# wns349/tensorflow-yolo

Hardware: AMD Instinct MI355X
Metric: images/sec at 1/2/4/8 MI355X + post-NMS box-set match vs CPU ref (higher is better)
Workload: dtype f16; 1 GPU; v3-608-b32-fp16; network=v3, batch_per_gpu=32, global_batch=32, weights=seeded synthetic Darknet stream (random-init), streams=1

## Files before the change

### tensorflow-yolo_amd/csrc/api.cpp

```cpp
#include <cstdio>
#include <cstring>
#include <new>

#include <cmath>
#include "yolo_internal.h"

namespace yolo {
const char *get_error();
}
using namespace yolo;

#define HIP_TRY(expr)                                                                          \
    do {                                                                                       \
        hipError_t e_ = (expr);                                                                \
        if (e_ != hipSuccess) {                                                                \
            set_error(std::string(#expr) + ": " + hipGetErrorString(e_));                      \
            return YOLO_ERR_HIP;                                                               \
        }                                                                                      \
    } while (0)

static int fail(int code, const std::string &msg) {
    set_error(msg);
    return code;
}
// ... 181 lines not shown
    }
    int esz(const View &v) const { return v.f32 ? 4 : net->esize; }
    unsigned char *view_ptr(const View &v) const { return buf_base(v.buf) + (size_t)(v.base + v.coff) * esz(v); }
};

void conv_vec_flags(const yolo_net *net, const Kernel &k, bool out_f32, int &vec_out, int &vec_res) {
    const int epc = net->epc;
    const int ch = k.cfg == CFG_N32 ? 8 : 16;
    const int oepc = out_f32 ? 4 : epc;
    vec_out = (k.cout % ch == 0) && (k.out.ld % oepc == 0) && ((k.out.base + k.out.coff) % oepc == 0) && (k.out.img_stride % oepc == 0);
    vec_res = k.has_res && (k.cout % ch == 0) && (k.in2.ld % epc == 0) && (k.in2.coff % epc == 0) && (k.in2.img_stride % epc == 0);
}

int make_conv_params(yolo_net *net, const Kernel &k, const Ptrs &P, int batch, ConvParams &p) {
    const int dtype = net->opt.dtype;
    memset(&p, 0, sizeof p);
    const View &in = k.in;
    const long long in_bytes = (long long)batch * in.img_stride * net->esize;
    if (in_bytes > 0x7ffffff0LL)
        return fail(YOLO_ERR_ARG, "conv input tensor exceeds 2 GiB (32-bit buffer addressing): lower the batch");
    p.in = P.buf_base(in.buf);
    p.in_bytes = (uint32_t)in_bytes;
    p.wgt = weights_at(net, k.w_off);
    p.wgt_bytes = (uint32_t)k.w_bytes;
    p.bias = reinterpret_cast<const float *>(weights_at(net, k.b_off));
    p.H = in.H; p.W = in.W; p.in_ld = in.ld; p.in_coff = in.coff; p.in_img_stride = in.img_stride;
    const yolo_layer_desc &d = net->layers[k.src_layer].d;
    const int Ho = net->layers[k.src_layer].H, Wo = net->layers[k.src_layer].W;
    p.Ho = Ho; p.Wo = Wo; p.HoWo = Ho * Wo;
    const long long M = (long long)batch * Ho * Wo;
    if (M > 0x7fffffffLL) return fail(YOLO_ERR_ARG, "too many output pixels for one launch");
    p.M = (int)M;
    p.Cout = k.cout;
    p.out = P.view_ptr(k.out);
    p.out_ld = k.out.ld;
    p.out_img_stride = k.out.img_stride;
    p.out_f32 = k.out.f32 || dtype == YOLO_DTYPE_F32;
    {
        const long long ob = (long long)batch * k.out.img_stride * (p.out_f32 ? 4 : net->esize);
        p.out_bytes = ob > 0 && ob <= 0x7ffffff0LL ? (uint32_t)ob : 0u;
    }
    p.ksize = d.ksize; p.stride = d.stride; p.pad = (d.ksize - 1) / 2; p.taps = d.ksize * d.ksize;
    p.ktiles = k.ktiles;
    p.tiles_per_tap = k.perchunk ? 1 : k.cpt / 8;
    p.cin_chunks = k.cpt;
    p.cpt_shift = k.cpt == 1 ? 0 : k.cpt == 2 ? 1 : 2;
    p.wrow_bytes = (uint32_t)k.ktiles * 128;
    p.leaky = k.leaky; p.outmode = k.outmode; p.has_res = k.has_res;
    p.f32 = dtype == YOLO_DTYPE_F32;
    int vo = 0, vr = 0;
    conv_vec_flags(net, k, p.out_f32 != 0, vo, vr);
    p.vec_out = vo && ((uintptr_t)P.buf_base(k.out.buf) % 16 == 0);
    if (k.head && net->obj_bytes && net->head.n_classes > 0 && !p.vec_out && p.out_f32 && k.outmode == OUT_NORMAL && !k.has_res) {
        const int width = 5 + net->head.n_classes;
        const long long base = k.out.base + k.out.coff;
        const size_t rows = net->out_count / (size_t)width;
        if (k.out.ld % width == 0 && base % width == 0 && rows * width == net->out_count && (size_t)batch * rows * 4 <= net->obj_bytes) {
            p.obj_out = reinterpret_cast<float *>(net->dev_ws + net->obj_off) + (size_t)P.img0 * rows;
            p.obj_width = width; p.obj_rows = (int)rows; p.obj_row0 = (int)(base / width); p.obj_na = k.out.ld / width;
            p.obj_min = net->obj_min_logit;
        }
    }
    if (k.has_res) {
        p.res = P.view_ptr(k.in2);
        p.res_ld = k.in2.ld;
        p.res_img_stride = k.in2.img_stride;
        const long long rbytes = (long long)batch * k.in2.img_stride * net->esize;
        p.res_bytes = rbytes > 0 && rbytes <= 0x7ffffff0LL ? (uint32_t)rbytes : 0u;
        p.vec_res = vr;
    }
    return YOLO_OK;
}

bool dma_eligible(const yolo_net *net, const Kernel &k) {
    if (k.cpt % 4) return false;
    return net->opt.dtype == YOLO_DTYPE_F16 || (k.ksize == 3 && k.stride == 1);
}
bool conv_tile_valid(const yolo_net *net, const Kernel &k, int tile) {
    if (k.outmode == OUT_POOL2 && tile != 12 && tile != 13 && tile != 17) return false;
    if (tile == 0) return true;
    if (net->opt.dtype == YOLO_DTYPE_F32 && !dma_cfg_f32_ok(tile)) return false;
    if ((tile == 18 || tile == 21 || tile == 22) && k.in.H != k.in.W) return false;
    if ((tile == 20 || tile == 21 || tile == 23) && ((k.in.H & 1) || net->opt.dtype != YOLO_DTYPE_F16)) return false;
    return dma_eligible(net, k) && dma_cfg_valid(tile, k.cout, k.cpt, true, k.ksize, k.stride, k.in.W);
}

int choose_ksplit(const Kernel &k, const ConvParams &p, int tile, size_t slab_bytes, int &ku) {
    ku = 0;
    if (!slab_bytes || p.M <= 0) return 1;
    long long blocks;
    int units, min_units;
    if (tile == 0) {
        const int na = k.cfg == CFG_N128 ? 128 : k.cfg == CFG_N64 ? 64 : 32, nb = k.cfg == CFG_N128 ? 128 : 256;
        blocks = ((long long)p.M + nb - 1) / nb * ((p.Cout + na - 1) / na);
        units = p.ktiles;
        min_units = 2;
    } else if (dma_cfg_is_tap(tile) && dma_cfg_splitk_ok(tile)) {
        const long long mq = (long long)(p.M / p.HoWo) * (p.H + 1) * (p.W + 1);
        blocks = (mq + dma_cfg_nb(tile) - 1) / dma_cfg_nb(tile) * ((p.Cout + dma_cfg_na(tile) - 1) / dma_cfg_na(tile));
        units = p.cin_chunks >> 2;
        min_units = 2;
    } else {
        return 1;
    }
    if (blocks > 128 || units < 2 * min_units) return 1;
    const long long kmax = units / min_units < 32 ? units / min_units : 32;
    long long ks = 512 / blocks;
    if (ks > kmax) ks = 256 / blocks;
    if (ks > kmax) ks = kmax;
    const size_t cout_pad = ((size_t)p.Cout + 127) / 128 * 128;
    const size_t wbytes = (size_t)p.Cout * (size_t)p.taps * (size_t)p.cin_chunks * 16;
    const size_t small_cap = (size_t)(p.taps == 1 ? 24 : (p.f32 || units >= 8) ? 16 : 8) << 20;
    while (ks >= 2 && ((size_t)ks * (size_t)p.M * cout_pad * 4 > slab_bytes || (size_t)ks * (size_t)p.M * cout_pad * 4 > (2 * wbytes > small_cap ? 2 * wbytes : small_cap))) --ks;
    if (ks < 2) return 1;
    ku = (int)((units + ks - 1) / ks);
    return (units + ku - 1) / ku;
}

struct ConvPick { int tile, ks, ku, pair; };
const size_t kSplitkSlabMax = (size_t)64 << 20;

ConvPick pick_conv(const yolo_net *net, const Kernel &k, const ConvParams &p, int tile_req, size_t slab_bytes) {
    int tile = tile_req;
    if (!dma_eligible(net, k) || (tile > 0 && !conv_tile_valid(net, k, tile))) tile = 0;
    else if (tile < 0) {
        tile = choose_dma_cfg(p.M, k.cout, k.cpt, p.taps, k.has_res, true, k.stride, k.in.W, net->opt.dtype == YOLO_DTYPE_F32);
        if (tile == 18 && !conv_tile_valid(net, k, 18)) tile = conv_tile_valid(net, k, 15) ? 15 : 8;
        if (tile == 22 && !conv_tile_valid(net, k, 22)) tile = conv_tile_valid(net, k, 10) ? 10 : 8;
        if ((tile == 20 || tile == 21) && !conv_tile_valid(net, k, tile)) tile = conv_tile_valid(net, k, 20) ? 20 : conv_tile_valid(net, k, 5) ? 5 : 0;
        if (tile == 23 && !conv_tile_valid(net, k, 23)) tile = conv_tile_valid(net, k, 6) ? 6 : 0;
    }
    static const bool no_pair_w = getenv("YOLO_NO_PAIR_SPLIT") != nullptr;
    bool wide_pair = false;
    if (tile > 0 && dma_cfg_is_tap(tile) && !no_pair_w && tile_req <= 0 && !p.f32 && (p.cin_chunks >> 2) >= 8 && p.HoWo > 0) {
        const long long mq = (long long)(p.M / p.HoWo) * (p.H + 1) * (p.W + 1);
        const long long ct = (p.Cout + 127) / 128;
        const long long b8 = (mq + 255) / 256 * ct, b22 = (long long)(p.M / p.HoWo) * ct;
        wide_pair = (conv_tile_valid(net, k, 22) && b22 >= 64 && b22 <= 128 && (size_t)b22 * 2 * 98304 <= slab_bytes) ||
                    (conv_tile_valid(net, k, 8) && b8 >= 64 && b8 <= 128 && (size_t)b8 * 2 * 131072 <= slab_bytes);
    }
    int ku = 0;
    int ks = wide_pair ? 1 : choose_ksplit(k, p, tile, slab_bytes, ku);
    if (ks <= 1 && !wide_pair && tile_req <= 0 && tile > 0 && dma_cfg_is_tap(tile) && tile != 11 && conv_tile_valid(net, k, 11)) {
        int ku11 = 0;
        const int ks11 = choose_ksplit(k, p, 11, slab_bytes, ku11);
        if (ks11 > 1) { tile = 11; ks = ks11; ku = ku11; }
    }
    int pair = 0;
    static const bool no_pair = getenv("YOLO_NO_PAIR_SPLIT") != nullptr;
    if (ks <= 1 && tile > 0 && dma_cfg_is_tap(tile) && !no_pair && tile_req <= 0) {
        const long long mq = (long long)(p.M / p.HoWo) * (p.H + 1) * (p.W + 1);
        const int units = p.cin_chunks >> 2;
        const long long ct = (p.Cout + 127) / 128;
        const long long b8 = (mq + 255) / 256 * ct, b11 = (mq + 127) / 128 * ct;
        const long long b22 = (long long)(p.M / p.HoWo) * ct;
        if (units >= 8 && !p.f32 && conv_tile_valid(net, k, 22) && b22 >= 64 && b22 <= 128 && (size_t)b22 * 2 * 98304 <= slab_bytes) {
            tile = 22; ks = 2; ku = (units + 1) / 2; pair = 1;
        } else if (units >= 8 && !p.f32 && conv_tile_valid(net, k, 8) && b8 >= 64 && b8 <= 128 && (size_t)b8 * 2 * 131072 <= slab_bytes) {
            tile = 8; ks = 2; ku = (units + 1) / 2; pair = 1;
        } else if (units >= 8 && conv_tile_valid(net, k, 11) && b11 > 128 && b11 <= 256 && (size_t)b11 * 2 * 65536 <= slab_bytes) {
            tile = 11; ks = 2; ku = (units + 1) / 2; pair = 1;
        }
    }
    static const bool no_inl = getenv("YOLO_NO_INLAUNCH_SPLITK") != nullptr;
    if (ks > 1 && ks <= 8 && !pair && tile == 11 && !no_inl) {
        const long long mq = (long long)(p.M / p.HoWo) * (p.H + 1) * (p.W + 1);
        const long long nb11 = (mq + 127) / 128 * ((p.Cout + 127) / 128);
        if (nb11 * 128 <= (long long)kPairCounterBytes && (size_t)nb11 * (size_t)ks * 65536 <= slab_bytes) pair = 1;
    }
    return ConvPick{tile, ks, ku, pair};
}

void conv_shape_params(const yolo_net *net, const Kernel &k, int batch, ConvParams &p) {
    memset(&p, 0, sizeof p);
    const yolo_layer_desc &d = net->layers[k.src_layer].d;
    p.H = k.in.H; p.W = k.in.W;
    p.Ho = net->layers[k.src_layer].H; p.Wo = net->layers[k.src_layer].W; p.HoWo = p.Ho * p.Wo;
    p.M = (int)((long long)batch * p.HoWo);
    p.Cout = k.cout;
    p.ksize = d.ksize; p.stride = d.stride; p.taps = d.ksize * d.ksize;
    p.ktiles = k.ktiles; p.cin_chunks = k.cpt;
    p.f32 = net->opt.dtype == YOLO_DTYPE_F32;
    p.out_f32 = k.out.f32 || p.f32;
    p.outmode = k.outmode; p.has_res = k.has_res;
    conv_vec_flags(net, k, p.out_f32 != 0, p.vec_out, p.vec_res);
    const long long ob = (long long)batch * k.out.img_stride * (p.out_f32 ? 4 : net->esize);
    p.out_bytes = ob > 0 && ob <= 0x7ffffff0LL ? (uint32_t)ob : 0u;
    const long long rb = k.has_res ? (long long)batch * k.in2.img_stride * net->esize : 0;
    p.res_bytes = rb > 0 && rb <= 0x7ffffff0LL ? (uint32_t)rb : 0u;
}

size_t splitk_slab_bytes(const yolo_net *net) {
    const int per = net->arena_full ? net->opt.max_batch : (net->opt.max_batch + net->arenas - 1) / net->arenas;
    size_t need = 0;
    for (const Kernel &k : net->kernels) {
        if (k.kind != K_CONV || k.stem >= 2) continue;
        for (int b = 1; b <= per; ++b) {
            ConvParams p;
            conv_shape_params(net, k, b, p);
            const ConvPick pk = pick_conv(net, k, p, k.tile, kSplitkSlabMax);
            if (pk.pair) {
                const long long mq = (long long)(p.M / p.HoWo) * (p.H + 1) * (p.W + 1);
                const int nb = dma_cfg_nb(pk.tile);
                const long long ptiles = pk.tile == 22 ? (long long)(p.M / p.HoWo) : (mq + nb - 1) / nb;
                const size_t bytes = (size_t)(ptiles * ((p.Cout + 127) / 128)) * (size_t)pk.ks * 128 * (size_t)nb * 4;
                if (bytes > need) need = bytes;
            } else if (pk.ks > 1) {
                const size_t bytes = (size_t)pk.ks * (size_t)p.M * (size_t)((p.Cout + 127) / 128 * 128) * 4;
                if (bytes > need) need = bytes;
            }
        }
    }
    return need ? kPairCounterBytes + (need + 4095) / 4096 * 4096 : 0;
// ... 742 lines not shown
```

### tensorflow-yolo_amd/csrc/conv_dma.hip

```cpp
#include "conv_common.h"
#include <cstdio>
#include <vector>

namespace yolo {

template <int N>
__device__ __forceinline__ void wait_vmcnt() {
    asm volatile("s_waitcnt vmcnt(%0)" ::"n"(N) : "memory");
}

typedef __attribute__((address_space(3))) void lds_void;

__device__ __forceinline__ void dma16(__amdgpu_buffer_rsrc_t rsrc, unsigned char *lds_dst, uint32_t voff) {
#if defined(__HIP_DEVICE_COMPILE__)
    __builtin_amdgcn_raw_ptr_buffer_load_lds(rsrc, (lds_void *)lds_dst, 16, voff, 0, 0, 0);
#else
    (void)rsrc; (void)lds_dst; (void)voff;
#endif
}

template <int BKC>
__device__ __forceinline__ int lds_swz(int r) {
    if (BKC == 8) return (r >> 1) & 7;
    return (0x78 >> (2 * ((r >> 2) & 3))) & 3;
// ... 136 lines not shown
            else wait_vmcnt<0>();
        } else {
            if (S >= 4 && after >= 2) wait_vmcnt<2 * JB>();
            else if (S >= 3 && after >= 1) wait_vmcnt<JB>();
            else wait_vmcnt<0>();
        }
        __builtin_amdgcn_sched_barrier(0);
        __builtin_amdgcn_s_barrier();
#ifdef YOLO_EXPERIMENT
        if (p.trace && kt == 0) t_first = wall_clock64();
        if (kt + S - 1 < KT && !(p.dbg & 1)) issue_tile(kt + S - 1, fill);
        if (!(p.dbg & 2)) compute(stage);
#else
        if (kt + S - 1 < KT) issue_tile(kt + S - 1, fill);
        compute(stage);
#endif
        stage = stage + 1 == S ? 0 : stage + 1;
        fill = fill + 1 == S ? 0 : fill + 1;
    }

#ifdef YOLO_EXPERIMENT
    if (p.dbg & 4) return;
    const unsigned long long t_loop = p.trace ? wall_clock64() : 0ull;
#endif
    if constexpr (FUSE2) {
        static_assert(!FUSE2 || (WM == 2 && WN == 4 && TM == 4 && TP == 4 && 2 * LDS_BYTES <= 163840), "back-to-back 1x1: 128 x 256 tile, two per CU");
        conv_epilogue_fused_1x1<0, false>(p, acc, m0, wm, wn, wave, lane, smem);
    } else
    if constexpr (EPI == 2) {
        static_assert(8 * 16 * kStagePitch(TM) * 4 + NB * kStageFlagAnchors * 4 <= S * TILE_BYTES, "staging slabs + row flags must fit in the ring");
        __syncthreads();
        conv_epilogue_f32_staged<TM, TP, 0, true, NB>(p, acc, n0 + wm * (TM * 16), m0 + wn * (TP * 16), lane,
                                         reinterpret_cast<float *>(smem) + wave * 16 * kStagePitch(TM),
                                         reinterpret_cast<float *>(smem) + 8 * 16 * kStagePitch(TM), wn * (TP * 16));
    } else if constexpr (EPI == 1) {
        conv_epilogue_fast<TM, TP, 0>(p, acc, n0 + wm * (TM * 16) + fq * CH, m0 + wn * (TP * 16), fr);
    } else {
        conv_epilogue<T, TM, TP, 0, true>(p, acc, n0 + wm * (TM * 16) + fq * CH, m0 + wn * (TP * 16), fr);
    }
#ifdef YOLO_EXPERIMENT
    if (p.trace && tid == 0) {
        asm volatile("s_waitcnt vmcnt(0)" ::: "memory");
        unsigned long long *r = p.trace + (size_t)blockIdx.x * 8;
        r[0] = t_start; r[1] = t_setup; r[2] = t_loop; r[3] = wall_clock64();
        r[4] = __builtin_amdgcn_s_getreg(0xF804);
        r[5] = __builtin_amdgcn_s_getreg(0xF814);
        r[6] = t_first;
        r[7] = (unsigned long long)clock64() - c_start;
    }
#endif
}

struct DmaCfg {
    int na, nb, slots_per_cu;
    float rate;
    const char *name;
    int bkc;
};
static const DmaCfg kCfgs[] = {
    {128, 128, 2, 0.55f, "", 8},
    {256, 256, 1, 0.80f, "256x256,K64,S2", 8},
    {256, 128, 1, 0.85f, "256x128,K64,S3", 8},
    {128, 256, 1, 0.85f, "128x256,K64,S3", 8},
    {256, 256, 1, 1.00f, "256x256,K32,S4", 4},
    {256, 128, 2, 1.30f, "256x128,K32,S3,x2", 4},
    {128, 256, 2, 1.30f, "128x256,K32,S3,x2", 4},
    {64, 512, 2, 1.00f, "64x512,K32,S2,x2", 4},
    {128, 256, 2, 1.00f, "128x256,tap9,x2", 4},
    {256, 256, 1, 1.00f, "256x256,tap9", 4},
    {128, 192, 2, 1.00f, "128x192,tap9,x2", 4},
    {128, 128, 2, 1.00f, "128x128,tap9,x2", 4},
    {128, 256, 2, 1.00f, "128x256,tap9,2d,x2", 4},
    {64, 256, 2, 1.00f, "64x256,tap9,2d,x2", 4},
    {128, 128, 3, 1.00f, "128x128,K32,S3,x3", 4},
    {256, 224, 1, 1.00f, "256x224,tap9", 4},
    {128, 128, 3, 1.00f, "128x128,tap9,2d,x3", 4},
    {32, 256, 2, 1.00f, "32x256,tap9,2d,x2", 4},
    {128, 384, 1, 1.00f, "128x384,tap9,img", 4},
    {128, 192, 1, 1.00f, "128x192,K64,S4", 8},
    {128, 256, 2, 1.00f, "128x256,tap9,s2,x2", 4},
    {128, 384, 1, 1.00f, "128x384,tap9,s2,img", 4},
    {128, 192, 2, 1.00f, "128x192,tap9,img,x2", 4},
    {128, 256, 2, 1.00f, "128x256,tap9,s2,wide,x2", 4},
};
static const int kNumCfgs = 24;
static const int kFirstTapCfg = 8, kLastTapCfg = 13;
static inline bool is_tap_cfg(int cfg) { return (cfg >= kFirstTapCfg && cfg <= kLastTapCfg) || (cfg >= 15 && cfg <= 18) || (cfg >= 20 && cfg <= 23); }
static inline int tap_variant(int cfg) { return cfg >= 20 ? cfg - 10 : cfg >= 15 ? cfg - 9 : cfg - kFirstTapCfg; }
bool dma_cfg_is_tap(int cfg) { return is_tap_cfg(cfg); }
bool dma_cfg_f32_ok(int cfg) { return is_tap_cfg(cfg) && conv_tap_f32_ok(tap_variant(cfg)); }

bool dma_cfg_valid(int cfg, int cout, int cin_chunks, bool v1_ok, int ksize, int stride, int W) {
    if (cfg == 0) return v1_ok;
    if (cfg < 0 || cfg >= kNumCfgs) return false;
    const DmaCfg &k = kCfgs[cfg];
    if (cin_chunks % k.bkc) return false;
    if (is_tap_cfg(cfg) && (ksize != 3 || stride != (conv_tap_stride2(tap_variant(cfg)) ? 2 : 1) || !conv_tap_fits(tap_variant(cfg), W))) return false;
    if (k.na == 32) return cout <= 32 && cout > 16;
    if (k.na == 64) return cout <= 64 && (!is_tap_cfg(cfg) || cout > 32);
    return k.na <= (cout + 127) / 128 * 128 && cout > 64;
}

struct TileCost { float a_shared, a_mid, a_alone, f; };
static const TileCost kCost[] = {
    {1.14f, 1.14f, 0.82f, 9.0f},
    {1.45f, 1.45f, 1.45f, 20.0f},
    {0.82f, 0.82f, 0.82f, 12.0f},
    {0.82f, 0.82f, 0.82f, 12.0f},
    {1.47f, 1.47f, 1.47f, 20.0f},
    {1.75f, 1.75f, 1.30f, 8.0f},
    {1.75f, 1.75f, 1.30f, 8.0f},
    {0.0f, 0.0f, 0.0f, 0.0f},
    {1.20f, 1.45f, 0.76f, 7.9f},
    {1.20f, 1.20f, 1.20f, 20.0f},
    {0.94f, 1.32f, 0.68f, 8.5f},
    {0.76f, 0.90f, 0.63f, 6.9f},
    {0.90f, 1.10f, 0.60f, 17.0f},
    {1.00f, 1.00f, 0.60f, 5.8f},
    {1.10f, 1.50f, 0.70f, 8.0f},
    {1.05f, 1.05f, 1.05f, 18.0f},
    {0.0f, 0.0f, 0.0f, 0.0f},
    {0.0f, 0.0f, 0.0f, 0.0f},
    {0.90f, 0.90f, 0.90f, 18.0f},
    {0.60f, 0.60f, 0.60f, 12.0f},
    {1.20f, 1.45f, 0.76f, 7.9f},
    {0.90f, 0.90f, 0.90f, 18.0f},
    {0.94f, 1.32f, 0.68f, 8.5f},
    {0.0f, 0.0f, 0.0f, 0.0f},
};

int choose_dma_cfg(int M, int cout, int cin_chunks, int taps, int has_res, bool v1_ok, int stride, int W, bool tap_only) {
    const int ksize = taps == 9 ? 3 : 1;
#ifdef YOLO_EXPERIMENT
    const char *force = getenv("YOLO_CONV_TILE");
    if (force && *force && dma_cfg_valid(atoi(force), cout, cin_chunks, v1_ok, ksize, stride, W) && (!tap_only || atoi(force) == 0 || is_tap_cfg(atoi(force))))
        return atoi(force);
#endif
    const int fallback = v1_ok ? 0 : -1;
    if (cout <= 32 && M >= 8192 && dma_cfg_valid(17, cout, cin_chunks, v1_ok, ksize, stride, W)) return 17;
    if (cout <= 64) {
        if (M >= 8192 && dma_cfg_valid(13, cout, cin_chunks, v1_ok, ksize, stride, W)) return 13;
        return !tap_only && dma_cfg_valid(7, cout, cin_chunks, v1_ok, ksize, stride, W) && M >= 8192 ? 7 : fallback;
    }
    if (!tap_only && taps == 9 && stride == 1 && W > 110 && cout <= 128 && cin_chunks <= 8 && M >= 262144 &&
        dma_cfg_valid(12, cout, cin_chunks, v1_ok, ksize, stride, W))
        return 12;
    if (!tap_only && taps == 9 && stride == 1 && W > 110 && cout <= 128 && cin_chunks <= 8 && M >= 65536 && M < 262144 &&
        dma_cfg_valid(16, cout, cin_chunks, v1_ok, ksize, stride, W))
        return 16;
    if (tap_only && v1_ok && taps == 9 && stride == 1 && W <= 14 && taps * cin_chunks * 4 >= 4608 &&
        ((long long)M * (W + 1) * (W + 1) / ((long long)W * W) + 127) / 128 * ((cout + 127) / 128) > 512)
        return 0;
    const double k64 = taps * cin_chunks / 8.0;
    int best = fallback;
    double best_t = 1e300;
    for (int c = 0; c < kNumCfgs; ++c) {
        if (tap_only && !dma_cfg_f32_ok(c)) continue;
        if (c == 12 && W <= 110) continue;
        const long long wg128 = (long long)((M + 127) / 128) * ((cout + 127) / 128);
        if (c == 14 && taps != 1 && !(stride == 2 && wg128 > 128 && wg128 <= 256)) continue;
        if (c == 19 && taps != 1) continue;
        if (c == 7 || c == 13 || c == 16 || c == 17 || c == 23 || !dma_cfg_valid(c, cout, cin_chunks, v1_ok, ksize, stride, W)) continue;
        const DmaCfg &k = kCfgs[c];
        long long Meff = M;
        const int Wq = is_tap_cfg(c) && conv_tap_stride2(tap_variant(c)) ? W / 2 : W;
        if (is_tap_cfg(c) && conv_tap_stride2(tap_variant(c))) {
            if (cin_chunks <= 8) continue;
            Meff = (long long)M * (Wq + 1) * (Wq + 1) / ((long long)Wq * Wq);
        } else if (is_tap_cfg(c)) {
            if (conv_tap_is2d(tap_variant(c))) { const long long th = k.nb / 16, tx = (W + 15) / 16, ty = (W + th - 1) / th; Meff = (long long)M * tx * ty * k.nb / ((long long)W * W); }
            else Meff = (long long)M * (W + 1) * (W + 1) / ((long long)W * W);
        }
        long long blocks = (Meff + k.nb - 1) / k.nb * ((cout + k.na - 1) / k.na);
        if (is_tap_cfg(c) && conv_tap_image_aligned(tap_variant(c))) blocks = (long long)(M / (Wq * Wq)) * ((cout + k.na - 1) / k.na);
        if (is_tap_cfg(c) && conv_tap_stride2(tap_variant(c)) && blocks <= 128) continue;
        const long long slots = 256LL * k.slots_per_cu;
        double rounds, a;
        if (k.slots_per_cu == 1) {
            rounds = (double)((blocks + slots - 1) / slots);
            a = kCost[c].a_shared;
        } else if (blocks > slots) {
            rounds = (double)blocks / slots + 0.5;
            a = kCost[c].a_shared;
        } else {
            rounds = 1.0;
            a = blocks <= 256 ? kCost[c].a_alone : kCost[c].a_mid;
        }
        const double t = rounds * (k64 * a + kCost[c].f * (has_res ? 1.0 : 0.7));
        if (t < best_t) { best_t = t; best = c; }
    }
    return best;
}

int dma_num_cfgs() { return kNumCfgs; }
int dma_cfg_na(int cfg) { return cfg > 0 && cfg < kNumCfgs ? kCfgs[cfg].na : 128; }
int dma_cfg_nb(int cfg) { return cfg > 0 && cfg < kNumCfgs ? kCfgs[cfg].nb : 128; }
bool dma_cfg_splitk_ok(int cfg) { return is_tap_cfg(cfg) && conv_tap_splitk_ok(tap_variant(cfg)); }
int dma_cfg_bkc(int cfg) { return cfg > 0 && cfg < kNumCfgs ? kCfgs[cfg].bkc : 8; }
const char *dma_cfg_name(int cfg) { return cfg > 0 && cfg < kNumCfgs ? kCfgs[cfg].name : ""; }

#define YOLO_DMA_VARIANTS(X) \
    X(1, 2, 4, 8, 4, 2, 8, 2) \
    X(2, 4, 2, 4, 4, 3, 8, 2) \
    X(3, 2, 4, 4, 4, 3, 8, 2) \
    X(4, 2, 4, 8, 4, 4, 4, 2) \
    X(5, 4, 2, 4, 4, 3, 4, 4) \
    X(6, 2, 4, 4, 4, 3, 4, 4) \
    X(7, 1, 8, 4, 4, 2, 4, 4) \
    X(14, 2, 4, 4, 2, 3, 4, 6) \
    X(19, 2, 4, 4, 3, 4, 8, 2)

static inline int dma_epilogue_kind(const ConvParams &p) {
    if (p.out_f32 && !p.vec_out && p.outmode == OUT_NORMAL && !p.has_res) return 2;
    static const bool no_fast_epi = getenv("YOLO_NO_FAST_EPI") != nullptr;
    return !no_fast_epi && conv_fast_epilogue_ok(p) ? 1 : 0;
}

static hipError_t launch_dma_tile(const ConvParams &p, int cfg, hipStream_t s) {
    const dim3 grid((unsigned)p.n_blocks), block(512);
    if (p.fuse2) {
        if (cfg != 6 || !conv_fast_epilogue_ok(p) || p.has_res || p.n_tiles_n != 1 || p.Cout != 128 || !p.w2 || !p.b2 || !p.out2 || !p.out2_bytes) return hipErrorInvalidValue;
        hipLaunchKernelGGL((conv_igemm_dma_kernel<2, 4, 4, 4, 3, 4, 4, true>), grid, block, 0, s, p);
        return hipGetLastError();
    }
    switch (cfg) {
#define X(id, ...) case id: \
        if (dma_epilogue_kind(p) == 2) hipLaunchKernelGGL((conv_igemm_dma_kernel<__VA_ARGS__, false, 2>), grid, block, 0, s, p); \
        else if (dma_epilogue_kind(p) == 1) hipLaunchKernelGGL((conv_igemm_dma_kernel<__VA_ARGS__, false, 1>), grid, block, 0, s, p); \
        else hipLaunchKernelGGL((conv_igemm_dma_kernel<__VA_ARGS__, false, 0>), grid, block, 0, s, p); \
        break;
        YOLO_DMA_VARIANTS(X)
#undef X
    default: return hipErrorInvalidValue;
    }
    return hipGetLastError();
}

#ifdef YOLO_EXPERIMENT
static hipError_t launch_traced(ConvParams p, int cfg, hipStream_t s) {
    const char *tf = getenv("YOLO_CONV_TRACE");
    unsigned long long *dev = nullptr;
    const size_t bytes = (size_t)p.n_blocks * 64;
    if (hipMalloc((void **)&dev, bytes) != hipSuccess) return hipErrorOutOfMemory;
    (void)hipMemset(dev, 0, bytes);
    p.trace = dev;
    hipError_t e = is_tap_cfg(cfg) ? launch_conv_tap(p, tap_variant(cfg), s) : launch_dma_tile(p, cfg, s);
    if (e == hipSuccess) e = hipStreamSynchronize(s);
    std::vector<unsigned long long> host((size_t)p.n_blocks * 8);
    if (e == hipSuccess) e = hipMemcpy(host.data(), dev, bytes, hipMemcpyDeviceToHost);
    (void)hipFree(dev);
    if (e == hipSuccess) {
        if (FILE *fp = fopen(tf, "ab")) {
            const unsigned long long hdr[8] = {(unsigned long long)p.n_blocks, (unsigned long long)p.M, (unsigned long long)p.Cout,
                                               (unsigned long long)p.cin_chunks, (unsigned long long)p.H, (unsigned long long)p.W,
                                               (unsigned long long)cfg, (unsigned long long)(p.ksize * 10 + p.stride)};
            fwrite(hdr, 8, 8, fp);
            fwrite(host.data(), 8, host.size(), fp);
            fclose(fp);
        }
    }
    return e;
}
#endif

hipError_t launch_conv_dma(const ConvParams &p0, int cfg, hipStream_t s) {
    if (cfg <= 0 || cfg >= kNumCfgs) return hipErrorInvalidValue;
    ConvParams p = p0;
    const DmaCfg &k = kCfgs[cfg];
#ifdef YOLO_EXPERIMENT
    { const char *d = getenv("YOLO_CONV_DBG"); p.dbg = d ? atoi(d) : 0; }
#endif
    p.n_tiles_n = (p.Cout + k.na - 1) / k.na;
    const long long blocks = ((long long)p.M + k.nb - 1) / k.nb * p.n_tiles_n;
    if (blocks <= 0 || blocks > 0x7fffffffLL) return hipErrorInvalidValue;
    p.n_blocks = (int)blocks;
    conv_set_divisors(p, p.cin_chunks / k.bkc);
    if (is_tap_cfg(cfg)) {
        long long mq;
        if (conv_tap_is2d(tap_variant(cfg))) {
            const int th = k.nb / 16;
            p.t2_shift = th == 16 ? 8 : 7;
            if (th != 16 && th != 8) return hipErrorInvalidValue;
            p.qW = (p.W + 15) / 16;
            p.qHW = p.qW * ((p.H + th - 1) / th);
            mq = (long long)(p.M / p.HoWo) * p.qHW * k.nb;
        } else {
            p.qW = p.Wo + 1;
            p.qHW = (p.Ho + 1) * (p.Wo + 1);
            mq = (long long)(p.M / p.HoWo) * p.qHW;
        }
        const bool img = conv_tap_image_aligned(tap_variant(cfg));
        p.q_stride = img ? p.qHW : k.nb;
        const long long qblocks = img ? (long long)(p.M / p.HoWo) * p.n_tiles_n : (mq + k.nb - 1) / k.nb * p.n_tiles_n;
        if (qblocks <= 0 || qblocks > 0x7fffffffLL) return hipErrorInvalidValue;
        p.Mq = (int)mq;
        p.n_blocks = (int)qblocks;
        conv_set_divisors(p, p.cin_chunks / k.bkc);
#ifdef YOLO_EXPERIMENT
        if (getenv("YOLO_CONV_TRACE")) return launch_traced(p, cfg, s);
#endif
        p.stream = 1;
#ifdef YOLO_EXPERIMENT
        if (getenv("YOLO_NO_TAP_STREAM")) p.stream = 0;
#endif
        return launch_conv_tap(p, tap_variant(cfg), s);
    }
#ifdef YOLO_EXPERIMENT
    if (getenv("YOLO_CONV_TRACE")) return launch_traced(p, cfg, s);
#endif
    return launch_dma_tile(p, cfg, s);
}

std::string dma_cfg_symbol_for(int cfg, bool f32, const ConvParams &p) {
    if (p.fuse2) return cfg == 6 ? "void yolo::conv_igemm_dma_kernel<2, 4, 4, 4, 3, 4, 4, true, 0>(yolo::ConvParams)"
                       : cfg == 23 ? "void yolo::conv3x3_tap_kernel<false, 2, 4, 4, 4, 26, 4, 4, false, true, true>(yolo::ConvParams)"
                                   : "void yolo::conv3x3_tap_kernel<false, 2, 4, 4, 4, 27, 4, 2, false, true, true>(yolo::ConvParams)";
    if (is_tap_cfg(cfg) && conv_tap_stream_ok(p, tap_variant(cfg))) return conv_tap_stream_symbol(tap_variant(cfg));
    if (!is_tap_cfg(cfg)) {
        std::string sym = dma_cfg_symbol(cfg, f32, false);
        const size_t at = sym.rfind(", false, 0>(");
        if (at != std::string::npos) sym[at + 9] = (char)('0' + dma_epilogue_kind(p));
        return sym;
    }
    std::string sym = dma_cfg_symbol(cfg, f32, !f32 && conv_fast_epilogue_ok(p) && cfg != 20 && cfg != 23);
    if (is_tap_cfg(cfg) && p.outmode == OUT_POOL2) {
        const size_t at = sym.rfind(", 2, false, false, false>(");
        if (at != std::string::npos) sym.replace(at, 26, ", 3, false, false, false>(");
    }
    return sym;
}

const char *dma_cfg_symbol(int cfg, bool f32, bool fast) {
    if (is_tap_cfg(cfg)) return conv_tap_symbol(tap_variant(cfg), f32, fast);
    switch (cfg) {
#define X(id, ...) case id: return fast ? "void yolo::conv_igemm_dma_kernel<" #__VA_ARGS__ ", false, 1>(yolo::ConvParams)" \
                                          : "void yolo::conv_igemm_dma_kernel<" #__VA_ARGS__ ", false, 0>(yolo::ConvParams)";
        YOLO_DMA_VARIANTS(X)
#undef X
    default: return "";
    }
}

}
```

### tensorflow-yolo_amd/csrc/yolo_internal.h

```cpp
#pragma once
#include <hip/hip_runtime.h>
#include <stdint.h>
#include <string>
#include <vector>

#include "yolo_hip.h"

namespace yolo {

enum OutMode { OUT_NORMAL = 0, OUT_UP2 = 1, OUT_REORG2 = 2, OUT_POOL2 = 3 };
enum BufId { BUF_NONE = -1, BUF_USER_OUT = -2, BUF_USER_IN = -3 };
enum ConvCfg { CFG_N128 = 0, CFG_N64 = 1, CFG_N32 = 2 };
enum KernelKind { K_PREP = 0, K_CONV = 1, K_POOL = 2, K_ELTWISE = 3, K_FIRST = 4 };

struct View {
    int buf = BUF_NONE;
    int H = 0, W = 0, C = 0;
    int ld = 0;
    int coff = 0;
    long long img_stride = 0;
    long long base = 0;
    bool f32 = false;
};

// ... 138 lines not shown
    uint32_t w2_bytes, wrow2;
    int H, W, Ho, Wo, out_ld;
    long long in_img_stride, out_img_stride;
    int tiles_x, tiles_y, n_tiles;
    FastDiv dtx, dty;
};

struct ResizeParams {
    const unsigned char *src;
    float *dst;
    int src_h, src_w, src_row_bytes, dst_h, dst_w, swap_rb;
};

struct PoolParams {
    const void *in;
    void *out;
    int H, W, C, in_ld, Ho, Wo, out_ld, stride;
    long long in_img_stride, out_img_stride;
    long long total;
};

struct EltParams {
    const void *a;
    const void *b;
    void *out;
    int H, W, C, a_ld, b_ld, out_ld, outmode, out_f32, a_f32;
    long long a_img_stride, b_img_stride, out_img_stride;
    long long total;
};

struct ReduceParams {
    const float *part;
    const float *bias;
    const void *res;
    void *out;
    float *obj_out;
    int obj_width, obj_rows, obj_row0, obj_na;
    int ksplit, M, Cout, cout_pad, HoWo, Wo;
    int out_ld, res_ld, leaky, outmode, out_f32, f32;
    long long out_img_stride, res_img_stride;
};

struct DecodeScale {
    int row0, h, w, na;
    double aw[YOLO_MAX_ANCHORS], ah[YOLO_MAX_ANCHORS];
};

struct DecodeParams {
    const float *logits;
    const float *obj;
    int version, n_classes, rows, n_scales;
    DecodeScale sc[YOLO_MAX_SCALES];
    float threshold;
    int cap;
    void *cand;
    int *cand_count;
    long long total_rows;
};

struct Candidate {
    float x, y;
    double w, h;
    float prob;
    int cls;
    unsigned scan;
    int pad_;
};

struct NmsParams {
    const Candidate *cand;
    const int *cand_count;
    int *reset_count;
    int cap, max_boxes, mode;
    double iou_threshold;
    yolo_box *boxes;
    int *counts;
    int *status;
    int *keep_idx;
    unsigned char *scratch;
    size_t scratch_stride;
};

hipError_t launch_conv(const ConvParams &p, int dtype, int cfg, bool perchunk, hipStream_t s);
int choose_dma_cfg(int M, int cout, int cin_chunks, int taps, int has_res, bool v1_ok, int stride, int W, bool tap_only = false);
bool dma_cfg_valid(int cfg, int cout, int cin_chunks, bool v1_ok, int ksize, int stride, int W);
bool dma_cfg_is_tap(int cfg);
int dma_cfg_bkc(int cfg);
hipError_t launch_conv_dma(const ConvParams &p, int cfg, hipStream_t s);
hipError_t launch_conv_tap(const ConvParams &p, int variant, hipStream_t s);
bool conv_tap_stream_ok(const ConvParams &p, int variant);
bool conv_tap_fits(int variant, int W);
bool conv_tap_is2d(int variant);
bool conv_tap_stride2(int variant);
bool conv_tap_image_aligned(int variant);
bool conv_tap_f32_ok(int variant);
bool dma_cfg_f32_ok(int cfg);
const char *dma_cfg_name(int cfg);
const char *dma_cfg_symbol(int cfg, bool f32, bool fast = false);
const char *conv_tap_symbol(int variant, bool f32, bool fast = false);
std::string dma_cfg_symbol_for(int cfg, bool f32, const ConvParams &p);
const char *conv_tap_stream_symbol(int variant);
std::string conv_symbol(int dtype, int cfg, bool perchunk, bool f32_emu = false);
bool conv_f32_emu_rule(int f32_products, int dtype, const ConvParams &p, int cfg, bool perchunk, int ksplit);
std::string first_symbol(int dtype, int cout, bool pool);
std::string aux_symbol(int kind, int dtype, bool vec);
int dma_num_cfgs();
int dma_cfg_na(int cfg);
int dma_cfg_nb(int cfg);
bool dma_cfg_splitk_ok(int cfg);
hipError_t launch_splitk_reduce(const ReduceParams &p, hipStream_t s);
bool conv_tap_splitk_ok(int variant);
bool conv_tap_pair_ok(int variant, bool f32);
hipError_t launch_prep(const PrepParams &p, int dtype, hipStream_t s);
hipError_t launch_resize(const ResizeParams &p, hipStream_t s);
hipError_t launch_first(const FirstParams &p, int dtype, hipStream_t s);
hipError_t launch_stem(const StemParams &p, int batch, hipStream_t s, int max_grid = 512);
hipError_t launch_pool(const PoolParams &p, int dtype, hipStream_t s);
hipError_t launch_eltwise(const EltParams &p, int dtype, hipStream_t s);
hipError_t launch_decode(const DecodeParams &p, int batch, hipStream_t s, bool zero_counts = true);
hipError_t launch_nms(const NmsParams &p, int batch, hipStream_t s);
size_t nms_lds_bytes(int cap);
size_t nms_scratch_bytes(int cap);

struct Kernel {
    int kind = 0;
    int layer = -1;
    int src_layer = -1;
    View in, in2, out;
    int ksize = 0, stride = 0, cout = 0, cin = 0, cin_s = 0, leaky = 0, outmode = 0, has_res = 0;
    int cfg = 0, perchunk = 0, cpt = 0, ktiles = 0;
    int tile = -1;
    int head = 0;
    int pool_fused = 0;
    int stem = 0;
    int fuse2_next = 0;
    int fuse2_prev = 0;
    int side = 0;
    size_t w_off = 0, b_off = 0, w_bytes = 0;
    size_t w_src = 0;
    int batch_norm = 0;
    int pool_stride = 0;
    std::string note;
};

struct LayerInfo {
    yolo_layer_desc d;
    int H = 0, W = 0, C = 0;
    std::vector<int> consumers;
    int fused_into = -1;
    View view;
    bool materialised = false;
};

}

struct yolo_net {
    yolo_net_options opt;
    std::vector<yolo::LayerInfo> layers;
    std::vector<yolo::Kernel> kernels;
    std::vector<yolo::Buffer> buffers;
    yolo_head_desc head;
    size_t weight_count = 0;
    size_t weights_bytes = 0;
    size_t act_bytes = 0;
    size_t logits_off = 0, cand_off = 0, count_off = 0, nms_off = 0;
    size_t splitk_off = 0, splitk_bytes = 0;
    size_t obj_off = 0, obj_bytes = 0;
    bool obj_valid = false;
    int cand_clean = 0;
    int side_chains = 0;
    std::vector<hipStream_t> branch;
    std::vector<hipEvent_t> e_bfork, e_bjoin;
// ... 28 lines not shown
```

Before: 6389 images/sec.

## Add persistent LDS-resident-weight streaming kernel for large 1x1 convolutions

Introduces a persistent 1x1 convolution kernel that loads the full weight slice into LDS once per workgroup and streams input pixel tiles through a multi-stage async buffer-load ring, with epilogues overlapped against in-flight loads. The tile chooser selects it for stride-1, non-residual f16 1x1 layers where Cout matches the slice width, K exceeds 256 and there are enough pixel tiles. The goal is to remove repeated weight reloads and per-tile launch/prologue cost of the generic GEMM tiles. The fixed grid of 256 workgroups and large LDS footprint limit occupancy, and applicability is narrow.

After: 6383 images/sec (median of 3 runs). Within noise of the previous version (-0.1%).

```diff
diff --git a/tensorflow-yolo_amd/csrc/api.cpp b/tensorflow-yolo_amd/csrc/api.cpp
--- a/tensorflow-yolo_amd/csrc/api.cpp
+++ b/tensorflow-yolo_amd/csrc/api.cpp
@@ -287,6 +287,7 @@
     if (net->opt.dtype == YOLO_DTYPE_F32 && !dma_cfg_f32_ok(tile)) return false;
     if ((tile == 18 || tile == 21 || tile == 22) && k.in.H != k.in.W) return false;
     if ((tile == 20 || tile == 21 || tile == 23) && ((k.in.H & 1) || net->opt.dtype != YOLO_DTYPE_F16)) return false;
+    if (tile == 24 && (k.has_res || k.out.f32 || net->opt.dtype != YOLO_DTYPE_F16)) return false;
     return dma_eligible(net, k) && dma_cfg_valid(tile, k.cout, k.cpt, true, k.ksize, k.stride, k.in.W);
 }
 
@@ -334,6 +335,8 @@
         if (tile == 22 && !conv_tile_valid(net, k, 22)) tile = conv_tile_valid(net, k, 10) ? 10 : 8;
         if ((tile == 20 || tile == 21) && !conv_tile_valid(net, k, tile)) tile = conv_tile_valid(net, k, 20) ? 20 : conv_tile_valid(net, k, 5) ? 5 : 0;
         if (tile == 23 && !conv_tile_valid(net, k, 23)) tile = conv_tile_valid(net, k, 6) ? 6 : 0;
+        if (tile == 24 && !conv_tile_valid(net, k, 24))
+            tile = choose_dma_cfg(p.M, k.cout, k.cpt, p.taps, k.has_res, true, k.stride, k.in.W, net->opt.dtype == YOLO_DTYPE_F32, true);
     }
     static const bool no_pair_w = getenv("YOLO_NO_PAIR_SPLIT") != nullptr;
     bool wide_pair = false;
diff --git a/tensorflow-yolo_amd/csrc/conv_1x1.hip b/tensorflow-yolo_amd/csrc/conv_1x1.hip
--- /dev/null
+++ b/tensorflow-yolo_amd/csrc/conv_1x1.hip
@@ -0,0 +1,235 @@
+#include "conv_common.h"
+
+namespace yolo {
+
+typedef __attribute__((address_space(3))) void c1_lds_void;
+
+template <int N>
+__device__ __forceinline__ void c1_wait_vmcnt() {
+    asm volatile("s_waitcnt vmcnt(%0)" ::"n"(N) : "memory");
+}
+
+__device__ __forceinline__ void c1_dma16(__amdgpu_buffer_rsrc_t rsrc, unsigned char *lds_dst, uint32_t voff) {
+#if defined(__HIP_DEVICE_COMPILE__)
+    __builtin_amdgcn_raw_ptr_buffer_load_lds(rsrc, (c1_lds_void *)lds_dst, 16, voff, 0, 0, 0);
+#else
+    (void)rsrc; (void)lds_dst; (void)voff;
+#endif
+}
+
+__device__ __forceinline__ int c1_swz(int r) { return (0x78 >> (2 * ((r >> 2) & 3))) & 3; }
+
+constexpr int kC1LdsBytes = 163840;
+constexpr int kC1Grid = 256;
+constexpr int kC1MaxSlices = 4;
+
+template <int WM, int WN, int TM, int TP, int S, int EPI>
+__global__ void __launch_bounds__(512, 2) conv1x1_stream_kernel(const ConvParams p) {
+    typedef _Float16 T;
+    static_assert(WM * WN == 8, "eight waves per workgroup");
+    constexpr int ROWB = 64;
+    constexpr int NA = WM * TM * 16;
+    constexpr int NB = WN * TP * 16;
+    constexpr int STAGE = NB * ROWB;
+    constexpr int WSTAGE = NA * ROWB;
+    constexpr int W_BYTES = kC1LdsBytes - S * STAGE;
+    constexpr int KT_MAX = W_BYTES / WSTAGE;
+    constexpr int JB = NB / 128;
+    constexpr int NWI = KT_MAX * (NA / 16) / 8;
+    constexpr int CH = 4 * TM;
+    constexpr int NST = TP * (CH / 8);
+    static_assert(JB >= 1 && NB % 128 == 0 && (KT_MAX * (NA / 16)) % 8 == 0 && S >= 3, "tile / wave mapping");
+    static_assert((S - 2) * JB + 2 * NST <= 63, "vmcnt range");
+    __shared__ __attribute__((aligned(16))) unsigned char smem[kC1LdsBytes];
+    unsigned char *const ring = smem + W_BYTES;
+
+    const int tid = threadIdx.x;
+    const int lane = tid & 63;
+    const int wave = __builtin_amdgcn_readfirstlane(tid >> 6);
+    const int wm = wave / WN, wn = wave % WN;
+    const int fr = lane & 15, fq = lane >> 4;
+
+    const int ns = p.n_tiles_n;
+    const int bx = blockIdx.x & 7, bt = blockIdx.x >> 3;
+    const int slice = bt % ns;
+    const int member = (bt / ns) * 8 + bx;
+    const int members = kC1Grid / ns;
+    const int n_ptiles = (p.M + NB - 1) / NB;
+    if (member >= n_ptiles) return;
+    const int my_tiles = (n_ptiles - 1 - member) / members + 1;
+    const int KT = p.cin_chunks >> 2;
+    const int G = my_tiles * KT;
+    const int n0 = slice * NA;
+
+    const __amdgpu_buffer_rsrc_t rs_in = __builtin_amdgcn_make_buffer_rsrc(const_cast<void *>(p.in), 0, p.in_bytes, 0x00020000);
+    const __amdgpu_buffer_rsrc_t rs_w = __builtin_amdgcn_make_buffer_rsrc(const_cast<void *>(p.wgt), 0, p.wgt_bytes, 0x00020000);
+
+    const int lrow = lane >> 2;
+    const uint32_t csw = (uint32_t)(((lane & 3) ^ c1_swz(lrow)) << 4);
+
+    float4v bv[TM];
+#pragma unroll
+    for (int a = 0; a < TM; ++a) bv[a] = *reinterpret_cast<const float4v *>(p.bias + n0 + wm * (TM * 16) + fq * CH + 4 * a);
+
+#pragma unroll
+    for (int jw = 0; jw < NWI; ++jw) {
+        const int i = jw * 8 + wave;
+        const int kt = i / (NA / 16), grp = i % (NA / 16);
+        const int r = grp * 16 + lrow;
+        const int ws = r / (TM * 16), R = r % (TM * 16);
+        const int tm = R >> 4, g4 = (R >> 2) & 3, jj = R & 3;
+        const int ch = ws * (TM * 16) + g4 * CH + 4 * tm + jj;
+        const uint32_t off = (uint32_t)(n0 + ch) * p.wrow_bytes + (uint32_t)kt * ROWB + csw;
+        c1_dma16(rs_w, smem + kt * WSTAGE + grp * 1024, kt < KT ? off : YOLO_INVALID_OFF);
+    }
+
+    int i_tile = member, i_kt = 0;
+    uint32_t b_base[JB];
+    auto geometry = [&]() __attribute__((always_inline)) {
+#pragma unroll
+        for (int j = 0; j < JB; ++j) {
+            const int m = i_tile * NB + (j * 8 + wave) * 16 + lrow;
+            const bool ok = i_tile < n_ptiles && m < p.M;
+            const int mm = ok ? m : 0;
+            const int n = (int)fdiv((uint32_t)mm, p.dHoWo);
+            const int rem = mm - n * p.HoWo;
+            const long long e = (long long)n * p.in_img_stride + (long long)rem * p.in_ld + p.in_coff;
+            b_base[j] = ok ? (uint32_t)(e * 2) + csw : YOLO_INVALID_OFF;
+        }
+    };
+    geometry();
+    auto issue = [&](int slot) __attribute__((always_inline)) {
+        const uint32_t koff = (uint32_t)i_kt * ROWB;
+#pragma unroll
+        for (int j = 0; j < JB; ++j) c1_dma16(rs_in, ring + slot * STAGE + (j * 8 + wave) * 1024, b_base[j] + koff);
+        if (++i_kt == KT) {
+            i_kt = 0;
+            i_tile += members;
+            geometry();
+        }
+    };
+
+    float4v acc[TM][TP];
+    auto init_acc = [&]() __attribute__((always_inline)) {
+#pragma unroll
+        for (int a = 0; a < TM; ++a)
+#pragma unroll
+            for (int b = 0; b < TP; ++b) acc[a][b] = bv[a];
+    };
+    const int so = ((fq ^ c1_swz(fr)) & 3) << 4;
+    auto compute = [&](int slot, int kt) __attribute__((always_inline)) {
+        const unsigned char *A = smem + kt * WSTAGE + (wm * TM * 16 + fr) * ROWB + so;
+        const unsigned char *B = ring + slot * STAGE + (wn * TP * 16 + fr) * ROWB + so;
+        uint4v fa[TM], fb[TP];
+#pragma unroll
+        for (int a = 0; a < TM; ++a) fa[a] = *reinterpret_cast<const uint4v *>(A + a * 16 * ROWB);
+#pragma unroll
+        for (int b = 0; b < TP; ++b) fb[b] = *reinterpret_cast<const uint4v *>(B + b * 16 * ROWB);
+#pragma unroll
+        for (int a = 0; a < TM; ++a)
+#pragma unroll
+            for (int b = 0; b < TP; ++b) acc[a][b] = mma_chunk<T>(fa[a], fb[b], acc[a][b]);
+    };
+
+#pragma unroll
+    for (int s = 0; s < S - 1; ++s) issue(s);
+    init_acc();
+    int slot = 0, fill = S - 1;
+    int c_kt = 0, m0 = member * NB;
+    int end1 = -S, end2 = -S;
+    for (int g = 0; g < G; ++g) {
+        const int lo = g - S + 1;
+        const int ne = EPI == 1 ? (end1 >= lo ? 1 : 0) + (end2 >= lo ? 1 : 0) : 0;
+        if (ne == 0) c1_wait_vmcnt<(S - 2) * JB>();
+        else if (ne == 1) c1_wait_vmcnt<(S - 2) * JB + NST>();
+        else c1_wait_vmcnt<(S - 2) * JB + 2 * NST>();
+        __builtin_amdgcn_sched_barrier(0);
+        __builtin_amdgcn_s_barrier();
+        issue(fill);
+        compute(slot, c_kt);
+        slot = slot + 1 == S ? 0 : slot + 1;
+        fill = fill + 1 == S ? 0 : fill + 1;
+        if (++c_kt == KT) {
+            if constexpr (EPI == 1) conv_epilogue_fast_body<TM, TP, 0, false>(p, acc, n0 + wm * (TM * 16) + fq * CH, m0 + wn * (TP * 16), fr);
+            else conv_epilogue<T, TM, TP, 0, true>(p, acc, n0 + wm * (TM * 16) + fq * CH, m0 + wn * (TP * 16), fr);
+            end2 = end1;
+            end1 = g;
+            c_kt = 0;
+            m0 += members * NB;
+            init_acc();
+        }
+    }
+    c1_wait_vmcnt<0>();
+}
+
+#define YOLO_C1_VARIANTS(X) \
+    X(0, 2, 4, 4, 2, 12) \
+    X(1, 2, 4, 4, 2, 8) \
+    X(2, 2, 4, 4, 2, 4) \
+    X(3, 1, 8, 4, 2, 6) \
+    X(4, 1, 8, 4, 2, 4)
+static const int kC1NA[] = {128, 128, 128, 64, 64};
+static const int kC1NB[] = {128, 128, 128, 256, 256};
+static const int kC1KMax[] = {256, 384, 512, 512, 768};
+static const int kC1Variants = 5;
+
+#ifndef YOLO_1X1_SLICE
+#define YOLO_1X1_SLICE 128
+#endif
+
+int conv1x1_stream_variant(int cout, int cin_chunks) {
+    const int K = cin_chunks * 8;
+    if (cout <= 0 || cout % 64 || cin_chunks % 4 || K <= 0) return -1;
+    const bool wide_first = cout == 128 || YOLO_1X1_SLICE >= 128;
+    for (int pass = 0; pass < 2; ++pass) {
+        const int na = (pass == 0) == wide_first ? 128 : 64;
+        for (int v = 0; v < kC1Variants; ++v)
+            if (kC1NA[v] == na && cout % na == 0 && cout / na <= kC1MaxSlices && K <= kC1KMax[v]) return v;
+    }
+    return -1;
+}
+
+bool conv1x1_stream_rule(int M, int cout, int cin_chunks) {
+    const int v = conv1x1_stream_variant(cout, cin_chunks);
+    return v >= 0 && kC1NA[v] == cout && cin_chunks * 8 > 256 && (M + kC1NB[v] - 1) / kC1NB[v] >= 2 * kC1Grid;
+}
+
+static inline int c1_epilogue_kind(const ConvParams &p) {
+    static const bool no_fast_epi = getenv("YOLO_NO_FAST_EPI") != nullptr;
+    return !no_fast_epi && conv_fast_epilogue_ok(p) ? 1 : 0;
+}
+
+hipError_t launch_conv1x1_stream(const ConvParams &p0, hipStream_t s) {
+    ConvParams p = p0;
+    const int v = conv1x1_stream_variant(p.Cout, p.cin_chunks);
+    if (v < 0 || p.ksize != 1 || p.stride != 1 || p.f32 || p.has_res || p.ksplit > 1 || p.fuse2 || p.Ho != p.H || p.Wo != p.W || p.M <= 0)
+        return hipErrorInvalidValue;
+    p.n_tiles_n = p.Cout / kC1NA[v];
+    p.n_blocks = kC1Grid;
+    conv_set_divisors(p, 1);
+    const dim3 grid(kC1Grid), block(512);
+    const bool lean = c1_epilogue_kind(p) == 1;
+    switch (v) {
+#define X(id, ...) case id: \
+        if (lean) hipLaunchKernelGGL((conv1x1_stream_kernel<__VA_ARGS__, 1>), grid, block, 0, s, p); \
+        else hipLaunchKernelGGL((conv1x1_stream_kernel<__VA_ARGS__, 0>), grid, block, 0, s, p); \
+        break;
+        YOLO_C1_VARIANTS(X)
+#undef X
+    default: return hipErrorInvalidValue;
+    }
+    return hipGetLastError();
+}
+
+std::string conv1x1_stream_symbol(const ConvParams &p) {
+    const int v = conv1x1_stream_variant(p.Cout, p.cin_chunks);
+    const char *epi = c1_epilogue_kind(p) == 1 ? ", 1>(yolo::ConvParams)" : ", 0>(yolo::ConvParams)";
+    switch (v) {
+#define X(id, ...) case id: return std::string("void yolo::conv1x1_stream_kernel<" #__VA_ARGS__) + epi;
+        YOLO_C1_VARIANTS(X)
+#undef X
+    default: return "";
+    }
+}
+
+}
diff --git a/tensorflow-yolo_amd/csrc/conv_dma.hip b/tensorflow-yolo_amd/csrc/conv_dma.hip
--- a/tensorflow-yolo_amd/csrc/conv_dma.hip
+++ b/tensorflow-yolo_amd/csrc/conv_dma.hip
@@ -242,8 +242,9 @@
     {128, 384, 1, 1.00f, "128x384,tap9,s2,img", 4},
     {128, 192, 2, 1.00f, "128x192,tap9,img,x2", 4},
     {128, 256, 2, 1.00f, "128x256,tap9,s2,wide,x2", 4},
+    {128, 128, 1, 1.00f, "1x1,stream", 4},
 };
-static const int kNumCfgs = 24;
+static const int kNumCfgs = 25;
 static const int kFirstTapCfg = 8, kLastTapCfg = 13;
 static inline bool is_tap_cfg(int cfg) { return (cfg >= kFirstTapCfg && cfg <= kLastTapCfg) || (cfg >= 15 && cfg <= 18) || (cfg >= 20 && cfg <= 23); }
 static inline int tap_variant(int cfg) { return cfg >= 20 ? cfg - 10 : cfg >= 15 ? cfg - 9 : cfg - kFirstTapCfg; }
@@ -253,6 +254,7 @@
 bool dma_cfg_valid(int cfg, int cout, int cin_chunks, bool v1_ok, int ksize, int stride, int W) {
     if (cfg == 0) return v1_ok;
     if (cfg < 0 || cfg >= kNumCfgs) return false;
+    if (cfg == 24) return ksize == 1 && stride == 1 && conv1x1_stream_variant(cout, cin_chunks) >= 0;
     const DmaCfg &k = kCfgs[cfg];
     if (cin_chunks % k.bkc) return false;
     if (is_tap_cfg(cfg) && (ksize != 3 || stride != (conv_tap_stride2(tap_variant(cfg)) ? 2 : 1) || !conv_tap_fits(tap_variant(cfg), W))) return false;
@@ -287,15 +289,20 @@
     {0.90f, 0.90f, 0.90f, 18.0f},
     {0.94f, 1.32f, 0.68f, 8.5f},
     {0.0f, 0.0f, 0.0f, 0.0f},
+    {0.0f, 0.0f, 0.0f, 0.0f},
 };
 
-int choose_dma_cfg(int M, int cout, int cin_chunks, int taps, int has_res, bool v1_ok, int stride, int W, bool tap_only) {
+int choose_dma_cfg(int M, int cout, int cin_chunks, int taps, int has_res, bool v1_ok, int stride, int W, bool tap_only, bool no_stream) {
     const int ksize = taps == 9 ? 3 : 1;
 #ifdef YOLO_EXPERIMENT
     const char *force = getenv("YOLO_CONV_TILE");
     if (force && *force && dma_cfg_valid(atoi(force), cout, cin_chunks, v1_ok, ksize, stride, W) && (!tap_only || atoi(force) == 0 || is_tap_cfg(atoi(force))))
         return atoi(force);
 #endif
+    static const bool no_1x1_stream = getenv("YOLO_NO_1X1_STREAM") != nullptr;
+    if (!no_1x1_stream && !no_stream && !tap_only && taps == 1 && stride == 1 && !has_res && dma_cfg_valid(24, cout, cin_chunks, v1_ok, ksize, stride, W) &&
+        conv1x1_stream_rule(M, cout, cin_chunks))
+        return 24;
     const int fallback = v1_ok ? 0 : -1;
     if (cout <= 32 && M >= 8192 && dma_cfg_valid(17, cout, cin_chunks, v1_ok, ksize, stride, W)) return 17;
     if (cout <= 64) {
@@ -320,7 +327,7 @@
         const long long wg128 = (long long)((M + 127) / 128) * ((cout + 127) / 128);
         if (c == 14 && taps != 1 && !(stride == 2 && wg128 > 128 && wg128 <= 256)) continue;
         if (c == 19 && taps != 1) continue;
-        if (c == 7 || c == 13 || c == 16 || c == 17 || c == 23 || !dma_cfg_valid(c, cout, cin_chunks, v1_ok, ksize, stride, W)) continue;
+        if (c == 7 || c == 13 || c == 16 || c == 17 || c == 23 || c == 24 || !dma_cfg_valid(c, cout, cin_chunks, v1_ok, ksize, stride, W)) continue;
         const DmaCfg &k = kCfgs[c];
         long long Meff = M;
         const int Wq = is_tap_cfg(c) && conv_tap_stride2(tap_variant(c)) ? W / 2 : W;
@@ -425,6 +432,7 @@
 
 hipError_t launch_conv_dma(const ConvParams &p0, int cfg, hipStream_t s) {
     if (cfg <= 0 || cfg >= kNumCfgs) return hipErrorInvalidValue;
+    if (cfg == 24) return launch_conv1x1_stream(p0, s);
     ConvParams p = p0;
     const DmaCfg &k = kCfgs[cfg];
 #ifdef YOLO_EXPERIMENT
@@ -475,6 +483,7 @@
     if (p.fuse2) return cfg == 6 ? "void yolo::conv_igemm_dma_kernel<2, 4, 4, 4, 3, 4, 4, true, 0>(yolo::ConvParams)"
                        : cfg == 23 ? "void yolo::conv3x3_tap_kernel<false, 2, 4, 4, 4, 26, 4, 4, false, true, true>(yolo::ConvParams)"
                                    : "void yolo::conv3x3_tap_kernel<false, 2, 4, 4, 4, 27, 4, 2, false, true, true>(yolo::ConvParams)";
+    if (cfg == 24) return conv1x1_stream_symbol(p);
     if (is_tap_cfg(cfg) && conv_tap_stream_ok(p, tap_variant(cfg))) return conv_tap_stream_symbol(tap_variant(cfg));
     if (!is_tap_cfg(cfg)) {
         std::string sym = dma_cfg_symbol(cfg, f32, false);
diff --git a/tensorflow-yolo_amd/csrc/yolo_internal.h b/tensorflow-yolo_amd/csrc/yolo_internal.h
--- a/tensorflow-yolo_amd/csrc/yolo_internal.h
+++ b/tensorflow-yolo_amd/csrc/yolo_internal.h
@@ -244,12 +244,17 @@
 };
 
 hipError_t launch_conv(const ConvParams &p, int dtype, int cfg, bool perchunk, hipStream_t s);
-int choose_dma_cfg(int M, int cout, int cin_chunks, int taps, int has_res, bool v1_ok, int stride, int W, bool tap_only = false);
+int choose_dma_cfg(int M, int cout, int cin_chunks, int taps, int has_res, bool v1_ok, int stride, int W, bool tap_only = false,
+                   bool no_stream = false);
 bool dma_cfg_valid(int cfg, int cout, int cin_chunks, bool v1_ok, int ksize, int stride, int W);
 bool dma_cfg_is_tap(int cfg);
 int dma_cfg_bkc(int cfg);
 hipError_t launch_conv_dma(const ConvParams &p, int cfg, hipStream_t s);
 hipError_t launch_conv_tap(const ConvParams &p, int variant, hipStream_t s);
+hipError_t launch_conv1x1_stream(const ConvParams &p, hipStream_t s);
+int conv1x1_stream_variant(int cout, int cin_chunks);
+bool conv1x1_stream_rule(int M, int cout, int cin_chunks);
+std::string conv1x1_stream_symbol(const ConvParams &p);
 bool conv_tap_stream_ok(const ConvParams &p, int variant);
 bool conv_tap_fits(int variant, int W);
 bool conv_tap_is2d(int variant);
```
